# 0Setsuna0/SoftbodyUnity

Measured on AMD Instinct MI355X. Metric: particle-substeps/sec, higher is better.
Workload: dtype f32

## Files before the change

softbodyunity_amd/csrc/abi.hip:

```cpp
#include "solver_internal.hpp"

using namespace sbi;

extern "C" {

void sb_desc_default(sb_desc *d) {
    if (!d) return;
    std::memset(d, 0, sizeof(*d));
    d->world = 1;
    d->gravity[1] = -9.81f;
    d->tile_particles = 0;
    d->use_graph = 1;
}

int sb_create(const sb_desc *desc, sb_solver **out) {
    if (!desc || !out) return fail(SB_ERR_INVALID_ARG, "sb_create: null argument");
    *out = nullptr;
    return guarded([&]() -> int {
        sb_desc d = *desc;
        if (d.world <= 0) d.world = 1;
        if (d.rank < 0 || d.rank >= d.world) return fail(SB_ERR_INVALID_ARG, "sb_create: rank out of range");
        if (!(d.damping >= 0.0f)) return fail(SB_ERR_INVALID_ARG, "sb_create: damping must be >= 0");
        if (d.tile_particles > sbp::kMaxTileLocal) return fail(SB_ERR_INVALID_ARG, "sb_create: tile_particles too large");
        if (d.partition < SB_PARTITION_AUTO || d.partition > SB_PARTITION_RCB) return fail(SB_ERR_INVALID_ARG, "sb_create: partition must be SB_PARTITION_AUTO, _BLOCKS or _RCB");
// ... 464 lines not shown
    return guarded([&]() -> int {
        int rc = set_device(s); if (rc) return rc;
        HIP_CHECK(hipEventRecord(s->ev1, s->stream));
        HIP_CHECK(hipEventSynchronize(s->ev1));
        HIP_CHECK(hipEventElapsedTime(ms, s->ev0, s->ev1));
        return SB_OK;
    });
}

int sb_get_stats(sb_solver *s, sb_stats *out) {
    if (!s || !out) return fail(SB_ERR_INVALID_ARG, "sb_get_stats: null argument");
    if (!s->finalized) return fail(SB_ERR_STATE, "sb_get_stats before sb_finalize");
    std::memset(out, 0, sizeof(*out));
    const sbp::Plan &P = s->plan->plan;
    const sbp::LocalPlan &L = s->plan->local;
    out->n_particles_owned = s->n_owned;
    out->n_particles_local = s->n_local;
    for (size_t k = 0; k < L.order_mask[0].size(); ++k) if (L.order_mask[0][k]) ++out->n_constraints_local[P.order_type[0][k]];
    out->n_tilings = P.tiling ? 2 : 1;
    out->n_global_colours = (int32_t)P.gcolours.size();
    for (int tl = 0; tl < 2; ++tl) { out->n_tiles[tl] = s->tiling[tl].n_tiles; out->tile_constraints[tl] = s->tiling[tl].n_slots; }
    out->n_t2_layers = (int64_t)s->t2_layer_range.size();
    out->n_t2_tiles = s->tiling[2].n_tiles;
    out->t2_constraints = s->tiling[2].n_slots;
    out->constraints_in_tiles = P.cons_in_tiles;
    out->constraints_in_global = P.cons_in_global;
    for (size_t slot = 0; slot < s->halos.size(); ++slot) {
        const int64_t cnt = s->halos[slot]->send_off.back();
        if (slot == 1) out->halo_particles_t1 = cnt; else out->halo_particles_global += cnt;
    }
    out->device_bytes = s->dev_bytes;
    {
        const int64_t mb = s->w_uniform ? 0 : (s->w_palette ? 1 : 4);
        auto tables = [&](const DevTiling &D) { return D.stream_bytes + (int64_t)D.n_tiles * (int64_t)sizeof(sbk::TileDesc) + (int64_t)D.runs_overflow.count * 8; };
        for (int tl = 0; tl < 2; ++tl) {
            const DevTiling &D = s->tiling[tl];
            if (!D.n_tiles) continue;
            out->launch_bytes[tl] = D.staged_particles * (12 + mb + 12 + 12 + 12) + tables(D);
        }
        const DevTiling &D0 = s->tiling[0];
        if (D0.n_tiles) {
            out->launch_bytes[2] = D0.staged_particles * (12 + mb + 12 + 12 + 12) + tables(D0);
            out->launch_bytes[3] = D0.staged_particles * (12 + mb + 12 + 12 + 12) + tables(D0);
        }
        const DevTiling &D2 = s->tiling[2];
        if (D2.n_tiles) out->launch_bytes[4] = D2.staged_particles * (4 + 12 + mb + 12) + tables(D2);
    }
    out->partition = P.partition;
    out->halo_schedule = s->schedule;
    out->halo_unpack_fused = s->fused_unpack ? 1 : 0;
    out->halo_auto_state = s->calib.state;
    out->halo_auto_ticks = s->calib.n[0] + s->calib.n[1];
    out->halo_auto_ms[0] = s->calib.decided_ms[0]; out->halo_auto_ms[1] = s->calib.decided_ms[1];
    out->readback_peeks = s->n_peeks;
    out->readback_peek_tiles = s->n_peek_tiles;
    out->ticks_fused = s->n_fused;
    out->ticks_fused_kinematic = s->n_kin_fused;
    for (int tl = 0; tl < 2; ++tl) out->lane_packed_tiles[tl] = s->tiling[tl].n_packed_tiles;
    out->plan_hash = s->plan_hash;
    if (!P.rank_cost.empty()) {
        out->partition_cost = P.rank_cost[(size_t)s->desc.rank];
        for (int64_t c : P.rank_cost) { out->partition_cost_total += c; out->partition_cost_max = std::max(out->partition_cost_max, c); }
    }
    {
        std::vector<uint8_t> is_peer((size_t)s->desc.world, 0);
        for (const auto &H : s->halos) {
            for (int pr : H->peers) is_peer[(size_t)pr] = 1;
            out->halo_particles_recv += H->recv_off.back();
        }
        for (uint8_t b : is_peer) out->halo_peers += b;
    }
    return SB_OK;
}

}
```

softbodyunity_amd/csrc/device_math.hip.hpp:

```cpp
#pragma once
#include "kernel_types.hpp"

namespace sbk {

__device__ __forceinline__ float4 pv_load(const PosView &P, int g) {
    const size_t o = 3 * (size_t)g;
    return make_float4(P.xyz[o], P.xyz[o + 1], P.xyz[o + 2], P.w[g]);
}
__device__ __forceinline__ void pv_store(const PosView &P, int g, const float4 &v) {
    const size_t o = 3 * (size_t)g;
    P.xyz[o] = v.x; P.xyz[o + 1] = v.y; P.xyz[o + 2] = v.z;
}

__device__ __forceinline__ void store3_through(float *p, float x, float y, float z) {
    f32x3_t v = {x, y, z};
    asm volatile("global_store_dwordx3 %0, %1, off sc0 sc1" ::"v"(p), "v"(v) : "memory");
}

struct V3 { float x, y, z; };
__device__ __forceinline__ V3 sub3(V3 a, V3 b) { return {a.x - b.x, a.y - b.y, a.z - b.z}; }
__device__ __forceinline__ V3 cross3(V3 a, V3 b) {
    float t0 = a.y * b.z, t1 = a.z * b.y, t2 = a.z * b.x, t3 = a.x * b.z, t4 = a.x * b.y, t5 = a.y * b.x;
    return {t0 - t1, t2 - t3, t4 - t5};
}
__device__ __forceinline__ float dot3(V3 a, V3 b) {
    float xx = a.x * b.x, yy = a.y * b.y, zz = a.z * b.z;
    return (xx + yy) + zz;
}
__device__ __forceinline__ V3 addscaled3(V3 x, float s, V3 g) {
    float a = s * g.x, b = s * g.y, c = s * g.z;
    return {x.x + a, x.y + b, x.z + c};
}
__device__ __forceinline__ V3 xyz(float4 p) { return {p.x, p.y, p.z}; }

__device__ __forceinline__ float sqrt_rn_normal(float x) {
#ifdef SB_LIBM_SQRT
    return sqrtf(x);
#endif
    float s = __builtin_amdgcn_sqrtf(x);
    float sd = __int_as_float(__float_as_int(s) - 1), su = __int_as_float(__float_as_int(s) + 1);
    float rd = __builtin_fmaf(-sd, s, x), ru = __builtin_fmaf(-su, s, x);
    s = rd <= 0.0f ? sd : s;
    return ru > 0.0f ? su : s;
}

__device__ __forceinline__ bool project_distance(float4 &a, float4 &b, float L0, float at) {
    float dx = a.x - b.x, dy = a.y - b.y, dz = a.z - b.z;
    float xx = dx * dx, yy = dy * dy, zz = dz * dz;
    float L2 = (xx + yy) + zz;
// ... 220 lines not shown
```

softbodyunity_amd/csrc/kernel_types.hpp:

```cpp
#pragma once
#include <hip/hip_runtime.h>
#include <stdint.h>

#include "stream_codec.hpp"

namespace sbk {

struct TickParams {
    float h, inv_h, hgx, hgy, hgz, kd, at_d, at_v, at_b;
    float pnx, pny, pnz, pd;
    int32_t plane_on;
    float pad[2];
};

constexpr int kKindFirst = 0, kKindMid = 1, kKindLast = 2, kKindLayer = 3, kKindPeek = 4, kKindMidKinematic = 5;
constexpr bool kind_is_kinematic(int k) { return k == kKindMidKinematic; }
constexpr int kind_base(int k) { return kind_is_kinematic(k) ? kKindMid : k; }
constexpr bool kind_has_mark(int k) { return k != kKindLayer; }
constexpr bool kind_rounds_before_mark(int k) { return k != kKindFirst; }
constexpr bool kind_rounds_after_mark(int k) { return k == kKindFirst || kind_base(k) == kKindMid; }
constexpr bool kind_ends_tick(int k) { return k == kKindLast || k == kKindPeek; }
constexpr bool kind_reads_prev(int k) { return kind_base(k) == kKindMid || k == kKindLast; }
constexpr bool kind_writes_peek(int k) { return k == kKindPeek; }
constexpr bool kind_may_read_ghosts(int k) { return k == kKindMid || k == kKindLast; }
constexpr bool kind_gathers(int k) { return k == kKindLayer; }

struct TileDesc {
    int32_t n_local, run_count, n_rounds;
    int32_t gather_begin;
    uint32_t s_begin;
    uint32_t s_hdr;
    uint32_t s_len;
    uint32_t packed_lanes;
    int32_t run_overflow;
    int32_t n_pal;
    int32_t n_steps;
    uint32_t s_items;
    int2 runs[10];
};
constexpr int kInlineRuns = 10;
constexpr int kWide8MaxTiles = 768;
#ifndef SB_REG_ROUNDS
#define SB_REG_ROUNDS 4
#endif
#ifndef SB_REG_ROUNDS_NARROW
#define SB_REG_ROUNDS_NARROW 3
#endif
constexpr int kRegRoundsWide = SB_REG_ROUNDS, kRegRoundsNarrow = SB_REG_ROUNDS_NARROW;
#ifdef SB_REG_COMPACT_ONLY
constexpr bool kRegFullSlots = false;
#else
constexpr bool kRegFullSlots = true;
#endif
constexpr bool kLanePackDecodable = kRegRoundsNarrow >= kLanePackRounds;
constexpr int kMaxRoundsLds = 128;

typedef float f32x3_t __attribute__((ext_vector_type(3)));
struct PosView {
    float *xyz;
    const float *w;
};

constexpr int kMaxMassPalette = 64;

struct TileArgs {
    PosView pos;
    const uint8_t *w8;
    const float *wpal;
    float *prev;
    float *vel;
    const TileDesc *tiles;
    const int2 *runs_overflow;
    const uint32_t *stream;
    const TickParams *tp;
    const int32_t *gather;
    int32_t max_local;
    int32_t rounds_dwords;
    int32_t pal_dwords;
    int32_t win_dwords;
    int32_t tile_base;
    int32_t w_uniform;
    int32_t item_waves;
    int32_t store_through;
    const float *ghost_src;
    int32_t n_owned;
    float *peek_out;
    const int32_t *kin_map;
    float *kin_target;
};
constexpr int kHaloNone = 0, kHaloGhosts = 1;

constexpr int kNarrowTileThreads = 128;
constexpr int kQuadTileThreads = 512;
constexpr int kWideTileThreads = 256;
constexpr int kRoundSlots = 256;
constexpr int kSmallTile = 512, kLargeTile = 1024;
typedef float f32x3 __attribute__((ext_vector_type(3)));

typedef float f32x4 __attribute__((ext_vector_type(4)));
typedef uint32_t u32x4 __attribute__((ext_vector_type(4)));

constexpr int kMaxPeers = 8;
struct PeerSlot {
    int32_t n_send, n_recv;
    int32_t send_off[kMaxPeers + 1];
    int32_t send_cap[kMaxPeers];
    float *remote_data[kMaxPeers];
    int32_t remote_stride[kMaxPeers];
    int32_t my_stride[kMaxPeers];
    int32_t recv_off[kMaxPeers + 1];
    int32_t recv_cnt[kMaxPeers];
    const float *my_data[kMaxPeers];
    uint32_t *remote_data_flag[kMaxPeers];
    uint32_t *my_ack_flag[kMaxPeers];
    uint32_t *my_data_flag[kMaxPeers];
    uint32_t *remote_ack_flag[kMaxPeers];
    uint32_t *local;
// ... 13 lines not shown
```

softbodyunity_amd/csrc/launch_shape.hpp:

```cpp
#pragma once
#include "kernel_types.hpp"
#include "tables_host.hpp"

namespace sbt {

struct LaunchShape { int threads, ppt; bool quads; };
inline bool same_width(const LaunchShape &a, const LaunchShape &b) { return a.threads == b.threads && a.ppt == b.ppt; }

constexpr LaunchShape kShapeNarrow{sbk::kNarrowTileThreads, sbk::kSmallTile / sbk::kNarrowTileThreads, false};
constexpr LaunchShape kShapeWide{sbk::kWideTileThreads, sbk::kSmallTile / sbk::kWideTileThreads, false};
constexpr LaunchShape kShapeWideLarge{sbk::kWideTileThreads, sbk::kLargeTile / sbk::kWideTileThreads, false};
constexpr LaunchShape kShapeEight{sbk::kQuadTileThreads, sbk::kSmallTile / sbk::kQuadTileThreads, false};
constexpr LaunchShape kShapeEightLarge{sbk::kQuadTileThreads, sbk::kLargeTile / sbk::kQuadTileThreads, false};

inline LaunchShape tile_launch_shape(const TilingScalars &D, int tile_lanes, int quad_lanes, int narrow_min_tiles, int n_tiles_in_launch, bool ghosts) {
    const bool small = D.max_local <= sbk::kSmallTile;
    const bool narrow = small && (D.packed_lanes ? D.packed_lanes == sbk::kLanePackLanes : (tile_lanes ? tile_lanes == sbk::kNarrowTileThreads : n_tiles_in_launch >= narrow_min_tiles));
    const bool quad8 = D.has_quads && quad_lanes == sbk::kQuadTileThreads;
    const bool wide8 = small && !D.has_quads && !D.packed_lanes && (tile_lanes ? tile_lanes == sbk::kQuadTileThreads : n_tiles_in_launch <= sbk::kWide8MaxTiles);
    const bool quads = ghosts ? false : D.has_quads;
    LaunchShape sh = quads && quad8 ? (small ? kShapeEight : kShapeEightLarge) : wide8 ? kShapeEight : narrow ? kShapeNarrow : small ? kShapeWide : kShapeWideLarge;
    sh.quads = quads;
    return sh;
}

}
```

softbodyunity_amd/csrc/schedule.hip:

```cpp
#include "solver_internal.hpp"
#include "launch_shape.hpp"
#include "tile_kernel.hip.hpp"
#include "aux_kernels.hip.hpp"

namespace sbi {

sbk::TickParams tick_params(const sb_solver *s, float dt, int substeps) {
    sbk::TickParams t{};
    volatile float S = (float)substeps;
    volatile float h = dt / S;
    t.h = h;
    volatile float inv_h = 1.0f / h;
    t.inv_h = inv_h;
    volatile float hx = h * s->desc.gravity[0], hy = h * s->desc.gravity[1], hz = h * s->desc.gravity[2];
    t.hgx = hx; t.hgy = hy; t.hgz = hz;
    volatile float td = s->desc.damping * h;
    volatile float kd = 1.0f - td;
    t.kd = kd < 0.0f ? 0.0f : (float)kd;
    volatile float h2 = h * h;
    volatile float ad = s->mesh->kind[0].compliance / h2;
    volatile float av = s->mesh->kind[1].compliance / h2;
    volatile float av36 = 36.0f * av;
    volatile float ab = s->mesh->kind[2].compliance / h2;
    t.at_d = ad; t.at_v = av36; t.at_b = ab;
// ... 128 lines not shown
    if (free_list.empty()) e.create(); else { e = std::move(free_list.back()); free_list.pop_back(); }
    HIP_CHECK(hipEventRecord(e, st));
    (join ? join_pending : pending).push_back(std::move(e));
}
void ExchangeTimer::recycle() {
    for (auto *v : {&pending, &join_pending}) {
        free_list.insert(free_list.end(), std::make_move_iterator(v->begin()), std::make_move_iterator(v->end()));
        v->clear();
    }
}

void halo_exchange(sb_solver *s, int slot, hipStream_t st) {
    if (!st) st = s->stream;
    if (!halo_slot_active(s, slot)) return;
    const bool timed = s->xtimer.enabled && !s->capturing;
    if (timed) s->xtimer.mark(st);
    if (!s->peer.enabled) halo_exchange_pre(s, slot, st);
    if (timed) s->xtimer.mark(st);
    if (s->peer.enabled) halo_exchange_pre(s, slot, st);
    if (!s->peer.enabled) {
        NCCL_CHECK(rccl().GroupStart());
        try {
            halo_exchange_calls(s, slot, st);
        } catch (...) {
            (void)rccl().GroupEnd();
            throw;
        }
        NCCL_CHECK(rccl().GroupEnd());
    }
    halo_exchange_post(s, slot, st);
    if (timed) s->xtimer.mark(st);
}

template <int KIND, bool Q, int THREADS, int PPT, bool W, int G>
void launch_tile_kernel(const sb_solver *s, const DevTiling &D, const sbk::TileDesc *tiles_at_base, int n_wg, const sbk::TileArgs &A) {
    hipLaunchKernelGGL((sbk::tile_kernel<KIND, Q, THREADS, PPT, W, G>), dim3(n_wg), dim3(THREADS), D.lds_bytes + s->lds_pad, s->stream, tiles_at_base, n_wg, A);
}
template <int KIND, bool Q, bool W, int G>
void launch_tile_shaped(const sb_solver *s, const DevTiling &D, const sbt::LaunchShape &sh, const sbk::TileDesc *tiles_at_base, int n_wg, const sbk::TileArgs &A) {
    using namespace sbt;
    if (same_width(sh, kShapeEight)) return launch_tile_kernel<KIND, Q, kShapeEight.threads, kShapeEight.ppt, W, G>(s, D, tiles_at_base, n_wg, A);
    if constexpr (Q) if (same_width(sh, kShapeEightLarge)) return launch_tile_kernel<KIND, Q, kShapeEightLarge.threads, kShapeEightLarge.ppt, W, G>(s, D, tiles_at_base, n_wg, A);
    if (same_width(sh, kShapeNarrow)) return launch_tile_kernel<KIND, Q, kShapeNarrow.threads, kShapeNarrow.ppt, W, G>(s, D, tiles_at_base, n_wg, A);
    if (same_width(sh, kShapeWide)) return launch_tile_kernel<KIND, Q, kShapeWide.threads, kShapeWide.ppt, W, G>(s, D, tiles_at_base, n_wg, A);
    if (same_width(sh, kShapeWideLarge)) return launch_tile_kernel<KIND, Q, kShapeWideLarge.threads, kShapeWideLarge.ppt, W, G>(s, D, tiles_at_base, n_wg, A);
    throw std::runtime_error("internal: no tile kernel is built for the launch shape asked for");
}

template <int KIND>
void launch_tile(sb_solver *s, DevTiling &D, int tile_begin = 0, int tile_end = -1, int halo = sbk::kHaloNone, const sbk::TileDesc *table = nullptr) {
    const bool ghosts = halo == sbk::kHaloGhosts;
    if (tile_end < 0) tile_end = D.n_tiles;
    if (tile_end <= tile_begin) return;
    sbk::TileArgs A{};
    A.pos = s->pos_view(); A.w8 = s->d_w8.p; A.wpal = s->d_wpal.p; A.prev = s->d_prev.p; A.vel = s->d_vel.p;
    A.tiles = D.tiles.p; A.runs_overflow = D.runs_overflow.p; A.stream = D.stream.p;
    A.tp = s->d_tp.p;
    A.gather = D.gather.p;
    A.w_uniform = s->w_uniform ? 1 : 0;
    A.item_waves = D.item_waves;
    A.store_through = tile_end - tile_begin <= s->store_through_max_tiles ? 3 : s->store_through_large;
    A.ghost_src = ghosts ? s->d_recvbuf.p : nullptr; A.n_owned = (int32_t)s->n_owned;
    A.peek_out = sbk::kind_writes_peek(KIND) ? s->d_peek.p : nullptr;
    A.kin_map = sbk::kind_is_kinematic(KIND) ? s->d_kin_map.p : nullptr; A.kin_target = sbk::kind_is_kinematic(KIND) ? s->d_kin_target.p : nullptr;
    A.max_local = D.max_local; A.win_dwords = D.win_dwords; A.tile_base = tile_begin; A.pal_dwords = D.pal_dwords; A.rounds_dwords = D.rounds_dwords;
    const sbk::TileDesc *tiles_at_base = table ? table : D.tiles.p + tile_begin;
    const int n_wg = tile_end - tile_begin;
    const sbt::LaunchShape sh = sbt::tile_launch_shape(D, s->tile_lanes, s->quad_lanes, s->narrow_min_tiles, n_wg, ghosts);
    constexpr bool kCanGhost = sbk::kind_may_read_ghosts(KIND);
    if (ghosts && !(kCanGhost && !D.has_quads)) throw std::runtime_error("internal: ghost-reading tile kernel requested for a launch that has none");
    const bool W = s->w_palette;
    if (ghosts) {
        if constexpr (kCanGhost) W ? launch_tile_shaped<KIND, false, true, sbk::kHaloGhosts>(s, D, sh, tiles_at_base, n_wg, A) : launch_tile_shaped<KIND, false, false, sbk::kHaloGhosts>(s, D, sh, tiles_at_base, n_wg, A);
    } else if (sh.quads) W ? launch_tile_shaped<KIND, true, true, sbk::kHaloNone>(s, D, sh, tiles_at_base, n_wg, A) : launch_tile_shaped<KIND, true, false, sbk::kHaloNone>(s, D, sh, tiles_at_base, n_wg, A);
    else W ? launch_tile_shaped<KIND, false, true, sbk::kHaloNone>(s, D, sh, tiles_at_base, n_wg, A) : launch_tile_shaped<KIND, false, false, sbk::kHaloNone>(s, D, sh, tiles_at_base, n_wg, A);
}

struct LaunchTimer {
    std::vector<Event> ev;
    std::vector<int> slot;
    hipStream_t stream;
    void begin(int which) {
        Event a, b;
        a.create(); b.create();
        HIP_CHECK(hipEventRecord(a, stream));
        ev.push_back(std::move(a)); ev.push_back(std::move(b)); slot.push_back(which);
    }
    void end() { HIP_CHECK(hipEventRecord(ev.back(), stream)); }
};

void launch_tick_kernel(sb_solver *s, int it, int substeps, LaunchTimer *lt, int tile_begin = 0, int tile_end = -1, bool kin = false) {
    const int tl = s->plan->plan.tiling ? (it & 1) : 0;
    DevTiling &D = s->tiling[tl];
    if (lt && D.n_tiles) lt->begin(it == 0 ? 2 + (int)s->gcolours.size() : (it == substeps ? 3 + (int)s->gcolours.size() : tl));
    const int halo_in = s->fused_unpack && tl == 1 ? sbk::kHaloGhosts : sbk::kHaloNone;
    if (it == 0) launch_tile<sbk::kKindFirst>(s, D, tile_begin, tile_end);
    else if (it < substeps && kin) launch_tile<sbk::kKindMidKinematic>(s, D, tile_begin, tile_end);
    else if (it < substeps) launch_tile<sbk::kKindMid>(s, D, tile_begin, tile_end, halo_in);
    else launch_tile<sbk::kKindLast>(s, D, tile_begin, tile_end, halo_in);
    if (lt && D.n_tiles) lt->end();
}

void launch_t2_layer(sb_solver *s, int layer, LaunchTimer *lt, bool with_halo = true) {
    const auto rg = s->t2_layer_range[layer];
// ... 434 lines not shown
```

softbodyunity_amd/csrc/solver_internal.hpp:

```cpp
#pragma once
#include <hip/hip_runtime.h>
#include <rccl/rccl.h>
#include <dlfcn.h>

#include <algorithm>
#include <array>
#include <atomic>
#include <chrono>
#include <climits>
#include <cmath>
#include <cstdio>
#include <cstdlib>
#include <cstring>
#include <limits>
#include <map>
#include <memory>
#include <mutex>
#include <type_traits>
#include <stdexcept>
#include <string>
#include <utility>
#include <vector>

#include "../../include/softbody.h"
// ... 108 lines not shown
struct sb_plan {
    sbp::Plan plan;
    sbp::LocalPlan local;
    bool owns_local = true;
};

struct sb_solver {
    sb_desc desc;
    bool finalized = false;
    sbi::Stream stream;
    sbi::Event ev0, ev1;
    ncclComm_t comm = nullptr;
    bool loopback = false;
    int schedule = SB_SCHEDULE_SERIAL_EAGER;
    uint64_t plan_hash = 0;
    sbi::Stream comm_stream;
    sbi::Event ev_boundary, ev_halo;
    bool overlap_halo = false;
    std::shared_ptr<sbi::AuthoredMesh> mesh = std::make_shared<sbi::AuthoredMesh>();
    bool sharded = false;
    sb_domain domain{};
    std::vector<int32_t> global_id;
    std::unique_ptr<sb_plan> plan;
    int64_t dev_bytes = 0;
    int64_t n_owned = 0, n_local = 0;
    DevBuf<float> d_pos3;
    DevBuf<float> d_wf;
    DevBuf<uint8_t> d_w8;
    DevBuf<float> d_wpal;
    bool w_palette = false;
    bool w_uniform = false;
    sbk::PosView pos_view() const { return sbk::PosView{d_pos3.p, d_wf.p}; }
    DevBuf<float> d_prev, d_vel;
    DevBuf<sbk::TickParams> d_tp;
    DevBuf<float> d_sendbuf, d_recvbuf;
    DevTiling tiling[3];
    std::vector<std::pair<int32_t, int32_t>> t2_layer_range;
    std::vector<std::unique_ptr<DevGColour>> gcolours;
    std::vector<std::unique_ptr<DevHalo>> halos;
    sbk::TickParams tp_host{};
    bool tp_valid = false;
    sbi::GraphCache graphs;
    bool deferred = false;
    int deferred_substeps = 0;
    uint32_t tune_flags = 0;
    int win_dwords_cap = 0;
    int prev_offset_bytes = 0;
    bool lazy_tick = true;
    int tile_lanes = 0;
    int quad_lanes = 512;
    int store_through_max_tiles = 6144;
    int store_through_large = 0;
    int narrow_min_tiles = 10240;
    size_t lds_pad = 0;
    bool pack_tiles = true;
    bool fused_unpack = false;
    bool graph_rccl = false;
    std::vector<float> h_stage;
    struct AutoSchedule {
        int state = 0;
        int tick = 0;
        sbi::Event ev[8];
        int n[2] = {0, 0};
        double decided_ms[2] = {0, 0};
    } calib;
    bool group_walk = false;
// ... 129 lines not shown
```

softbodyunity_amd/csrc/tables.hip:

```cpp
#include "solver_internal.hpp"

namespace sbi {

sbp::Input make_input(const float *rest, int32_t n, const int32_t *d, int64_t md, const int32_t *v, int64_t mv,
                      const int32_t *b, int64_t mb) {
    sbp::Input in;
    in.rest = rest; in.n = n; in.dist_ij = d; in.m_d = md; in.vol = v; in.m_v = mv; in.bend = b; in.m_b = mb;
    return in;
}

sbp::Domain to_domain(const sb_domain &d) {
    sbp::Domain D;
    D.set = true; D.n_global = d.n_global; D.ell = d.spacing; D.fill = d.fill > 0 && d.fill <= 1 ? d.fill : 1.0;
    for (int a = 0; a < 3; ++a) { D.lo[a] = d.lo[a]; D.hi[a] = d.hi[a]; }
    return D;
}
sbp::Opts plan_opts(int rank, int world, const int32_t dims[3], int32_t tile_particles, int32_t partition, uint32_t plan_flags,
                    int64_t m_v, int64_t m_b, const sb_domain *domain) {
    sbp::Opts o;
    if (domain) {
        o.domain = to_domain(*domain);
        if (domain->four_vertex_constraints) m_v += 1;
    }
    o.rank = rank; o.world = world <= 0 ? 1 : world;
    for (int a = 0; a < 3; ++a) o.dims[a] = dims ? dims[a] : 0;
    o.tile_particles = tile_particles != 0 ? tile_particles : (m_v + m_b > 0 ? 256 : 512);
    o.partition = partition;
    o.third_tiling = !(plan_flags & SB_PLAN_NO_T2);
    o.third_list = !(plan_flags & SB_PLAN_NO_THIRD_LIST);
    o.cluster_layers = !(plan_flags & SB_PLAN_NO_CLUSTER_LAYERS);
    o.mixed_groups = !(plan_flags & SB_PLAN_NO_MIXED_GROUPS);
    o.bank_aware_lanes = !(plan_flags & SB_PLAN_NO_BANK_ORDER);
    o.merge_tiles = !(plan_flags & SB_PLAN_NO_TILE_MERGE);
// ... 75 lines not shown
    HIP_CHECK(hipMemset(s->d_prev.p, 0, (size_t)s->n_local * 3 * sizeof(float)));
    s->d_tp.alloc(1, s->dev_bytes);
    for (int tl = 0; tl < 3; ++tl) {
        sbt::build_tiling(in, opt, tl, H);
        sbt::HostTiling &T = H.T[tl];
        DevTiling &D = s->tiling[tl];
        static_cast<sbt::TilingScalars &>(D) = T;
        D.tiles.upload(T.tiles, s->dev_bytes); D.runs_overflow.upload(T.runs_overflow, s->dev_bytes);
        D.stream.upload(T.stream, s->dev_bytes);
        D.gather.upload(T.gather, s->dev_bytes);
        T.release_arrays();
    }
    s->t2_layer_range = H.t2_layer_range;
    sbt::build_gcolours(in, H);
    for (const sbt::HostGColour &G : H.gcolours) {
        auto D = std::make_unique<DevGColour>();
        D->type = G.type; D->count = G.count;
        if (G.type == 0) { D->ij.upload(G.ij, s->dev_bytes); D->rest.upload(G.rest, s->dev_bytes); }
        else { D->quad.upload(G.quad, s->dev_bytes); D->rest2.upload(G.rest2, s->dev_bytes); }
        s->gcolours.push_back(std::move(D));
    }
    sbt::build_halos(in, opt, H);
    for (sbt::HostHalo &G : H.halos) {
        auto D = std::make_unique<DevHalo>();
        D->send_idx.upload(G.send_idx, s->dev_bytes); D->recv_idx.upload(G.recv_idx, s->dev_bytes);
        D->peers = std::move(G.peers); D->send_off = std::move(G.send_off); D->recv_off = std::move(G.recv_off);
        s->halos.push_back(std::move(D));
    }
    s->d_sendbuf.alloc(H.send_floats, s->dev_bytes);
    s->d_recvbuf.alloc(H.recv_floats, s->dev_bytes);
    if (H.recv_floats) HIP_CHECK(hipMemset(s->d_recvbuf.p, 0, H.recv_floats * sizeof(float)));
    s->fused_unpack = H.fused_unpack;
    if (s->peer.enabled && L.world > 1) alloc_mailbox(s, H.mailbox);
}

}
```

softbodyunity_amd/csrc/tile_kernel.hip.hpp:

```cpp
#pragma once
#include "device_math.hip.hpp"

namespace sbk {

__device__ __forceinline__ void lds_barrier() { asm volatile("s_waitcnt lgkmcnt(0)\n\ts_barrier" ::: "memory"); }

__device__ __forceinline__ void decode_compact_distance(uint32_t e, const float *s_pal, int &i, int &k, float &L0) { i = compact_slot_i(e); k = compact_slot_j(e); L0 = s_pal[compact_slot_pal(e)]; }
__device__ __forceinline__ void decode_full_distance(const uint2 e, int &i, int &k, float &L0) { i = pair_i(e.x); k = pair_j(e.x); L0 = __uint_as_float(e.y); }
__device__ __forceinline__ void read_distance_slot(const uint32_t *slots, int c, bool compact, const float *s_pal, int &i, int &k, float &L0) {
    if (compact) decode_compact_distance(slots[c], s_pal, i, k, L0);
    else decode_full_distance(*reinterpret_cast<const uint2 *>(slots + kFullSlotDwords * c), i, k, L0);
}

__device__ __forceinline__ void quad_slot_offsets(const uint4 &e, int q, int &o0, int &o1, int &o2, int &o3) {
    o0 = 4 * (int)pair_i(e.x) + q; o1 = 4 * (int)pair_j(e.x) + q;
    o2 = 4 * (int)pair_i(e.y) + q; o3 = 4 * (int)pair_j(e.y) + q;
}

template <bool QUADS, int THREADS> constexpr int kWavesPerSimd = QUADS ? (THREADS == 64 ? 3 : (THREADS == 512 ? 2 : 4)) : (THREADS == 256 ? 8 : (THREADS == 128 ? 6 : 4));
template <int KIND_, bool QUADS, int THREADS, int PPT, bool WPAL, int HALO = kHaloNone>
__global__ __launch_bounds__(THREADS, (kWavesPerSimd<QUADS, THREADS> - (KIND_ == 5 && !QUADS ? 1 : 0))) void tile_kernel(const TileDesc *tiles_at_base, int n_workgroups, TileArgs A) {
    constexpr int KIND = kind_base(KIND_);
    constexpr bool KIN = kind_is_kinematic(KIND_);
    constexpr bool GHOSTS = HALO == kHaloGhosts;
    constexpr int kTileThreads = THREADS;
    constexpr int kCPL = THREADS >= kRoundSlots ? 1 : kRoundSlots / THREADS;
    extern __shared__ uint4 lds_raw[];
    float4 *lds_pos = reinterpret_cast<float4 *>(lds_raw);
    uint32_t *s_rounds = reinterpret_cast<uint32_t *>(lds_pos + A.max_local);
    float *s_pal = reinterpret_cast<float *>(s_rounds + A.rounds_dwords);
    uint32_t *cbuf = s_rounds + A.rounds_dwords + A.pal_dwords;
    f32x3 *lds_spare = reinterpret_cast<f32x3 *>(cbuf + A.win_dwords);
    typedef const TileDesc __attribute__((address_space(4))) *ConstTileDescPtr;
#ifndef SB_NO_XCD_REMAP
    const int nwg = n_workgroups, wg = (int)blockIdx.x;
    const int xq = nwg >> 3, xr = nwg & 7, xcd = wg & 7;
    const int tile_index = (xcd < xr ? xcd * (xq + 1) : xr * (xq + 1) + (xcd - xr) * xq) + (wg >> 3);
#else
    const int tile_index = (int)blockIdx.x;
#endif
    const TileDesc __attribute__((address_space(4))) &td = *((ConstTileDescPtr)(uintptr_t)tiles_at_base + tile_index);
    const int n_rounds_all = td.n_rounds;
    const int tid = threadIdx.x;
    const int n_local = td.n_local;
    const int run_count = td.run_count;
    const TickParams tp = *A.tp;
    const uint32_t *tstream = A.stream + td.s_begin;
#if defined(SB_ABLATE) && SB_ABLATE == 4
    if (n_local >= 0) { if (n_rounds_all == 0x7fffffff) A.vel[0] = tp.h; return; }
#endif

    int g[PPT];
    if (kind_gathers(KIND_)) {
// ... 19 lines not shown
                    if (rn.y <= l) gi = rn.x + (l - rn.y);
                }
            g[m] = l < n_local ? gi : -1;
        }
    }
    const int R = n_rounds_all;
    const int v_begin = kind_rounds_before_mark(KIND_) ? 0 : R;
    const int v_end = !kind_has_mark(KIND_) ? R : (kind_rounds_after_mark(KIND_) ? 2 * R + 1 : R + 1);
    const uint32_t d_lo = td.s_hdr;
    const uint32_t d_hi = td.s_len;
    const uint32_t win = (uint32_t)A.win_dwords;
    uint32_t win_lo = d_lo;
    auto load_window = [&](uint32_t lo) {
        const uint32_t n4 = (min(lo + win, d_hi) - lo) >> 2;
        const uint4 *src = reinterpret_cast<const uint4 *>(tstream + lo);
        uint4 *dst = reinterpret_cast<uint4 *>(cbuf);
        uint32_t t0 = (uint32_t)tid;
        asm volatile("" : "+v"(t0));
        for (uint32_t i = t0; i < n4; i += 4 * kTileThreads) {
            uint4 v0 = src[i], v1, v2, v3;
            const bool b1 = i + kTileThreads < n4, b2 = i + 2 * kTileThreads < n4, b3 = i + 3 * kTileThreads < n4;
            if (b1) v1 = src[i + kTileThreads];
            if (b2) v2 = src[i + 2 * kTileThreads];
            if (b3) v3 = src[i + 3 * kTileThreads];
            dst[i] = v0;
            if (b1) dst[i + kTileThreads] = v1;
            if (b2) dst[i + 2 * kTileThreads] = v2;
            if (b3) dst[i + 3 * kTileThreads] = v3;
        }
    };
    f32x4 X[PPT];
    float pvx[PPT], pvy[PPT], pvz[PPT];
    uint32_t wi[PPT];
    const int mypal = WPAL ? __float_as_int(A.wpal[tid & (kMaxMassPalette - 1)]) : 0;
#pragma unroll
    for (int m = 0; m < PPT; ++m) {
        const int gc = max(g[m], 0);
        const bool ghost = GHOSTS && gc >= A.n_owned;
        const float *px = ghost ? A.ghost_src + 6 * (size_t)(gc - A.n_owned) : A.pos.xyz + 3 * (size_t)gc;
        X[m].x = px[0]; X[m].y = px[1]; X[m].z = px[2];
        if (WPAL) { wi[m] = A.w8[A.w_uniform ? 0 : gc]; X[m].w = 0.0f; } else { wi[m] = 0; X[m].w = A.pos.w[gc]; }
        pvx[m] = pvy[m] = pvz[m] = 0.0f;
        if (kind_reads_prev(KIND_)) {
            const float *pp = ghost ? px + 3 : A.prev + 3 * (size_t)gc;
            pvx[m] = pp[0]; pvy[m] = pp[1]; pvz[m] = pp[2];
        }
    }
    const bool rounds_in_lds = n_rounds_all <= A.rounds_dwords;
    const uint32_t rw = tstream[max(min(tid, n_rounds_all - 1), 0)];
    const bool rounds_in_lanes = n_rounds_all <= 64;
    const uint32_t rwl = tstream[max(min(tid & 63, n_rounds_all - 1), 0)];
    uint32_t itreg = 0;
    if (QUADS && kTileThreads == 64 * A.item_waves) {
        const int ns = td.n_steps;
        itreg = tstream[ns > 0 ? td.s_items + (uint32_t)((tid >> 6) * ns + min(tid & 63, ns - 1)) : 0u];
    }
    const int n_pal = td.n_pal;
    const uint32_t palw = tstream[tid < n_pal ? ((n_rounds_all + 3) & ~3) + tid : 0];
#ifndef SB_KW
#define SB_KW (QUADS ? 4 : 2)
#endif
    constexpr int kW = SB_KW;
    const bool lane_packed = !QUADS && kTileThreads == kLanePackLanes && td.packed_lanes == (uint32_t)kLanePackLanes;
    const bool lane_packed_full = !WPAL && lane_packed && td.n_pal == 0;
    const bool wide_packed = !QUADS && kTileThreads == kWidePackLanes && td.packed_lanes == (uint32_t)kWidePackLanes;
    const bool any_packed = lane_packed || wide_packed;
    const uint32_t n4_first = wide_packed ? 0u : lane_packed ? (lane_packed_full ? 2u * (uint32_t)kLanePackLanes : (uint32_t)kLanePackLanes)
                                          : (min(win_lo + win, d_hi) - win_lo) >> 2;
    const u32x4 *wsrc = reinterpret_cast<const u32x4 *>(tstream + win_lo);
    u32x4 wv[kW];
#pragma unroll
    for (int q = 0; q < kW; ++q) {
        const uint32_t i = tid + q * kTileThreads;
        wv[q] = i < n4_first ? wsrc[i] : *reinterpret_cast<const u32x4 *>(tstream);
    }
    typedef uint32_t u32x2 __attribute__((ext_vector_type(2)));
    u32x2 wc = {0u, 0u};
    u32x2 wp = {0u, 0u};
    if (!QUADS && kTileThreads == kWidePackLanes)
        wp = *reinterpret_cast<const u32x2 *>(wide_packed ? tstream + win_lo + 2u * (uint32_t)tid : tstream);
#pragma unroll
    for (int m = 0; m < PPT; ++m) asm volatile("" ::"v"(X[m].x), "v"(pvx[m]), "v"(wi[m]), "v"(X[m].w));
    asm volatile("" ::"v"(mypal));
    if (WPAL) {
#pragma unroll
        for (int m = 0; m < PPT; ++m) X[m].w = __int_as_float(__builtin_amdgcn_ds_bpermute((int)(wi[m] << 2), mypal));
    }
#pragma unroll
    for (int q = 0; q < kW; ++q) asm volatile("" ::"v"(wv[q].x));
    asm volatile("" ::"v"(rw), "v"(palw), "v"(rwl), "v"(itreg));
    if (!QUADS && kTileThreads == kWidePackLanes) asm volatile("" ::"v"(wp.x));
#pragma unroll
    for (int m = 0; m < PPT; ++m)
        if (g[m] >= 0) *reinterpret_cast<f32x4 *>(lds_pos + tid + m * kTileThreads) = X[m];
    if (rounds_in_lds && tid < n_rounds_all) s_rounds[tid] = rw;
    if (tid < n_pal) s_pal[tid] = __uint_as_float(palw);
    if (kTileThreads < kMaxRoundsLds && rounds_in_lds)
        for (int q = tid + kTileThreads; q < n_rounds_all; q += kTileThreads) s_rounds[q] = tstream[q];
    if (kTileThreads < kMaxPalette)
        for (int q = tid + kTileThreads; q < n_pal; q += kTileThreads) s_pal[q] = __uint_as_float(tstream[((n_rounds_all + 3) & ~3) + q]);
    {
        u32x4 *dst = reinterpret_cast<u32x4 *>(cbuf);
#pragma unroll
        for (int q = 0; q < kW; ++q) {
            const uint32_t i = tid + q * kTileThreads;
            if (i < n4_first && !any_packed) dst[i] = wv[q];
        }
        if (!any_packed)
            for (uint32_t i = tid + kW * kTileThreads; i < n4_first; i += kTileThreads) dst[i] = wsrc[i];
    }
    __syncthreads();
    if (!WPAL && !QUADS && kTileThreads == kLanePackLanes && lane_packed_full)
        wc = *reinterpret_cast<const u32x2 *>(tstream + win_lo + 8u * (uint32_t)kLanePackLanes + 2u * (uint32_t)tid);
#if defined(SB_ABLATE) && SB_ABLATE == 5
    if (n_local >= 0) { if (lds_pos[tid].x == 1.2345e-30f && cbuf[tid] == 0x12345678u) A.vel[0] = tp.h; return; }
#endif
// ... 5 lines not shown
                const int l = tid + m * kTileThreads;
                float4 P = lds_pos[l];
                if (KIND != kKindFirst && tp.plane_on && P.w > 0.0f) {
                    float a = tp.pnx * P.x, b = tp.pny * P.y, c = tp.pnz * P.z;
                    float pen = ((a + b) + c) - tp.pd;
                    if (pen < 0.0f) {
                        float dx = pen * tp.pnx, dy = pen * tp.pny, dz = pen * tp.pnz;
                        P.x = P.x - dx; P.y = P.y - dy; P.z = P.z - dz;
                        if (kind_ends_tick(KIND_)) lds_pos[l] = P;
                    }
                }
                if (KIND == kKindPeek) continue;
                float vx, vy, vz;
                const size_t o = 3 * (size_t)g[m];
                if (KIND == kKindFirst) {
                    vx = A.vel[o + 0]; vy = A.vel[o + 1]; vz = A.vel[o + 2];
                } else {
                    float dx = P.x - pvx[m], dy = P.y - pvy[m], dz = P.z - pvz[m];
                    float qx = dx * tp.inv_h, qy = dy * tp.inv_h, qz = dz * tp.inv_h;
                    vx = qx * tp.kd; vy = qy * tp.kd; vz = qz * tp.kd;
                }
                bool moved = false;
                if (KIN && P.w == 0.0f) {
                    const int ks = A.kin_map[g[m]];
                    if (ks >= 0) {
                        float *t = A.kin_target + 3 * (size_t)ks;
                        const float tx = t[0], ty = t[1], tz = t[2];
                        if (tx == tx) { P.x = tx; P.y = ty; P.z = tz; moved = true; t[0] = __int_as_float(0x7fc00000); }
                    }
                }
                if (KIND == kKindLast) {
                    A.vel[o + 0] = vx; A.vel[o + 1] = vy; A.vel[o + 2] = vz;
                } else {
                    if (A.store_through & 1) store3_through(A.prev + o, P.x, P.y, P.z);
                    else { A.prev[o + 0] = P.x; A.prev[o + 1] = P.y; A.prev[o + 2] = P.z; }
                    if (P.w > 0.0f) {
                        vx = vx + tp.hgx; vy = vy + tp.hgy; vz = vz + tp.hgz;
                        float hx = tp.h * vx, hy = tp.h * vy, hz = tp.h * vz;
                        P.x = P.x + hx; P.y = P.y + hy; P.z = P.z + hz;
                        lds_pos[l] = P;
                    } else if (KIN && moved) lds_pos[l] = P;
                }
            }
    };

    constexpr int kRegRounds = THREADS >= 256 ? kRegRoundsWide : kRegRoundsNarrow;
    if (kRegRounds > 0 && !QUADS && n_rounds_all <= kRegRounds && n_rounds_all > 0 && (kRegFullSlots || n_pal > 0) && (any_packed || d_hi - d_lo <= win)) {
        const bool tile_compact = n_pal > 0;
        uint32_t rs[kRegRounds > 0 ? kRegRounds : 1][kCPL];
        float rl[kRegRounds > 0 ? kRegRounds : 1][kCPL];
        int rcnt[kRegRounds > 0 ? kRegRounds : 1];
        {
            uint32_t o = 0;
#pragma unroll
            for (int r = 0; r < kRegRounds; ++r) {
                rcnt[r] = 0;
                if (r < n_rounds_all) {
                    rcnt[r] = (int)group_dist_count((uint32_t)__builtin_amdgcn_readlane((int)rwl, r));
                    if (kCPL == 2 && lane_packed) {
#pragma unroll
                        for (int u = 0; u < kCPL; ++u) {
                            const int bit = kLanePackFieldBits * (2 * r + u), w0 = bit >> 5, sh = bit & 31;
                            const uint32_t lo = wv[0][w0] >> sh;
                            const uint32_t hi = (sh + kLanePackFieldBits > 32) ? (wv[0][w0 + 1 < kLaneWordDwords ? w0 + 1 : kLaneWordDwords - 1] << ((32 - sh) & 31)) : 0u;
                            const uint32_t f = (lo | hi) & kLanePackFieldMask;
                            rs[r][u] = compact_slot_of_pack_field(f);
                            if (!WPAL) {
// ... 249 lines not shown
            for (int u = 0; u < kCPL; ++u) {
                ca[u] = *reinterpret_cast<const f32x4 *>(lds_pos + ci[u]);
                cb[u] = *reinterpret_cast<const f32x4 *>(lds_pos + ck[u]);
            }
#pragma unroll
            for (int u = 0; u < kCPL; ++u) {
                float4 a = make_float4(ca[u].x, ca[u].y, ca[u].z, ca[u].w), b = make_float4(cb[u].x, cb[u].y, cb[u].z, cb[u].w);
                con[u] = project_distance_nobranch(a, b, cL0[u], tp.at_d) && con[u];
                ca[u].x = a.x; ca[u].y = a.y; ca[u].z = a.z; cb[u].x = b.x; cb[u].y = b.y; cb[u].z = b.z;
            }
#pragma unroll
            for (int u = 0; u < kCPL; ++u) {
                f32x3 *da = con[u] ? reinterpret_cast<f32x3 *>(lds_pos + ci[u]) : lds_spare;
                f32x3 *db = con[u] ? reinterpret_cast<f32x3 *>(lds_pos + ck[u]) : lds_spare;
                *da = (f32x3){ca[u].x, ca[u].y, ca[u].z};
                *db = (f32x3){cb[u].x, cb[u].y, cb[u].z};
            }
        }
        off += size;
#if defined(SB_ABLATE) && SB_ABLATE == 3
        asm volatile("s_waitcnt lgkmcnt(0)" ::: "memory");
#else
        lds_barrier();
#endif
    }
    }
#pragma unroll
    for (int m = 0; m < PPT; ++m)
        if (g[m] >= 0) {
            const float4 P = lds_pos[tid + m * kTileThreads];
            if (kind_writes_peek(KIND_)) { float *o = A.peek_out + 3 * (size_t)g[m]; o[0] = P.x; o[1] = P.y; o[2] = P.z; }
            else if (A.store_through & 2) store3_through(A.pos.xyz + 3 * (size_t)g[m], P.x, P.y, P.z);
            else pv_store(A.pos, g[m], P);
        }
}


}
```

Before: 115.4 billion.

## Encode previous positions as 64-bit bit-deltas against current positions

Replaces the 12-byte previous-position array with an 8-byte code per particle. The code packs 21-bit signed deltas between the float bit patterns of the previous and current positions, with an escape flag that falls back to the full-precision prev array when a delta does not fit. It is enabled only for single-rank, palette-mass, narrow spring-only tilings with no intermediate steps, and aims to cut memory traffic in the bandwidth-bound tile kernels. The cost is extra encode/decode ALU work, a divergent fallback path, and a restricted set of configurations where it applies.

```diff
diff --git a/softbodyunity_amd/csrc/abi.hip b/softbodyunity_amd/csrc/abi.hip
--- a/softbodyunity_amd/csrc/abi.hip
+++ b/softbodyunity_amd/csrc/abi.hip
@@ -520,16 +520,17 @@
     out->device_bytes = s->dev_bytes;
     {
         const int64_t mb = s->w_uniform ? 0 : (s->w_palette ? 1 : 4);
+        const int64_t pb = s->prev_codes ? 8 : 12;
         auto tables = [&](const DevTiling &D) { return D.stream_bytes + (int64_t)D.n_tiles * (int64_t)sizeof(sbk::TileDesc) + (int64_t)D.runs_overflow.count * 8; };
         for (int tl = 0; tl < 2; ++tl) {
             const DevTiling &D = s->tiling[tl];
             if (!D.n_tiles) continue;
-            out->launch_bytes[tl] = D.staged_particles * (12 + mb + 12 + 12 + 12) + tables(D);
+            out->launch_bytes[tl] = D.staged_particles * (12 + mb + pb + 12 + pb) + tables(D);
         }
         const DevTiling &D0 = s->tiling[0];
         if (D0.n_tiles) {
-            out->launch_bytes[2] = D0.staged_particles * (12 + mb + 12 + 12 + 12) + tables(D0);
-            out->launch_bytes[3] = D0.staged_particles * (12 + mb + 12 + 12 + 12) + tables(D0);
+            out->launch_bytes[2] = D0.staged_particles * (12 + mb + 12 + 12 + pb) + tables(D0);
+            out->launch_bytes[3] = D0.staged_particles * (12 + mb + pb + 12 + 12) + tables(D0);
         }
         const DevTiling &D2 = s->tiling[2];
         if (D2.n_tiles) out->launch_bytes[4] = D2.staged_particles * (4 + 12 + mb + 12) + tables(D2);
diff --git a/softbodyunity_amd/csrc/device_math.hip.hpp b/softbodyunity_amd/csrc/device_math.hip.hpp
--- a/softbodyunity_amd/csrc/device_math.hip.hpp
+++ b/softbodyunity_amd/csrc/device_math.hip.hpp
@@ -15,6 +15,10 @@
 __device__ __forceinline__ void store3_through(float *p, float x, float y, float z) {
     f32x3_t v = {x, y, z};
     asm volatile("global_store_dwordx3 %0, %1, off sc0 sc1" ::"v"(p), "v"(v) : "memory");
+}
+typedef uint32_t u32x2_t __attribute__((ext_vector_type(2)));
+__device__ __forceinline__ void store2_through(uint2 *p, u32x2_t v) {
+    asm volatile("global_store_dwordx2 %0, %1, off sc0 sc1" ::"v"(p), "v"(v) : "memory");
 }
 
 struct V3 { float x, y, z; };
diff --git a/softbodyunity_amd/csrc/kernel_types.hpp b/softbodyunity_amd/csrc/kernel_types.hpp
--- a/softbodyunity_amd/csrc/kernel_types.hpp
+++ b/softbodyunity_amd/csrc/kernel_types.hpp
@@ -21,6 +21,7 @@
 constexpr bool kind_rounds_after_mark(int k) { return k == kKindFirst || kind_base(k) == kKindMid; }
 constexpr bool kind_ends_tick(int k) { return k == kKindLast || k == kKindPeek; }
 constexpr bool kind_reads_prev(int k) { return kind_base(k) == kKindMid || k == kKindLast; }
+constexpr bool kind_touches_prev(int k) { return k == kKindFirst || kind_reads_prev(k); }
 constexpr bool kind_writes_peek(int k) { return k == kKindPeek; }
 constexpr bool kind_may_read_ghosts(int k) { return k == kKindMid || k == kKindLast; }
 constexpr bool kind_gathers(int k) { return k == kKindLayer; }
@@ -82,7 +83,10 @@
     int32_t w_uniform;
     int32_t item_waves;
     int32_t store_through;
-    const float *ghost_src;
+    union {
+        const float *ghost_src;
+        uint2 *prev_code;
+    };
     int32_t n_owned;
     float *peek_out;
     const int32_t *kin_map;
diff --git a/softbodyunity_amd/csrc/launch_shape.hpp b/softbodyunity_amd/csrc/launch_shape.hpp
--- a/softbodyunity_amd/csrc/launch_shape.hpp
+++ b/softbodyunity_amd/csrc/launch_shape.hpp
@@ -24,4 +24,25 @@
     return sh;
 }
 
+inline bool tiling_always_narrow(const TilingScalars &D, int tile_lanes) {
+    if (D.n_tiles == 0) return true;
+    return D.max_local <= sbk::kSmallTile && !D.has_quads && (D.packed_lanes ? D.packed_lanes == sbk::kLanePackLanes : tile_lanes == sbk::kNarrowTileThreads);
 }
+constexpr int64_t kPrevCodeMaxParticles = (int64_t)1 << 26;
+struct PrevCodeInputs {
+    int world = 1;
+    int halo_slots = 0;
+    int tile_lanes = 0;
+    bool w_palette = false;
+    int steps_between_tiles = 0;
+    int64_t n_local = 0;
+};
+inline bool use_prev_codes(const TilingScalars &T0, const TilingScalars &T1, const PrevCodeInputs &in) {
+    if (in.world != 1 || in.halo_slots != 0) return false;
+    if (!in.w_palette) return false;
+    if (in.steps_between_tiles != 0) return false;
+    if (T0.n_tiles == 0 || in.n_local > kPrevCodeMaxParticles) return false;
+    return tiling_always_narrow(T0, in.tile_lanes) && tiling_always_narrow(T1, in.tile_lanes);
+}
+
+}
diff --git a/softbodyunity_amd/csrc/prev_code.hpp b/softbodyunity_amd/csrc/prev_code.hpp
--- /dev/null
+++ b/softbodyunity_amd/csrc/prev_code.hpp
@@ -0,0 +1,34 @@
+#pragma once
+#include <stdint.h>
+
+#ifdef __HIPCC__
+#define SB_PREV_FN __host__ __device__ __forceinline__
+#else
+#define SB_PREV_FN inline
+#endif
+
+namespace sbk {
+
+constexpr int kPrevFieldBits = 21;
+constexpr uint32_t kPrevFieldMask = (1u << kPrevFieldBits) - 1u, kPrevHalf = 1u << (kPrevFieldBits - 1);
+constexpr uint64_t kPrevEscape = 1ull << 63;
+
+struct Bits3 { uint32_t x, y, z; };
+struct PrevCode { uint64_t code; bool fits; };
+
+SB_PREV_FN bool prev_delta_fits(uint32_t k) { return k + kPrevHalf < 2u * kPrevHalf; }
+SB_PREV_FN bool prev_is_escape(uint64_t code) { return (code >> 63) != 0; }
+SB_PREV_FN bool prev_hi_is_escape(uint32_t code_hi) { return (code_hi >> 31) != 0; }
+SB_PREV_FN PrevCode prev_encode(Bits3 P, Bits3 x) {
+    const uint32_t kx = P.x - x.x, ky = P.y - x.y, kz = P.z - x.z;
+    const bool fits = prev_delta_fits(kx) && prev_delta_fits(ky) && prev_delta_fits(kz);
+    const uint64_t f = (uint64_t)(kx & kPrevFieldMask) | ((uint64_t)(ky & kPrevFieldMask) << kPrevFieldBits) | ((uint64_t)(kz & kPrevFieldMask) << (2 * kPrevFieldBits));
+    return {fits ? f : kPrevEscape, fits};
+}
+SB_PREV_FN uint32_t prev_field_delta(uint32_t f) { return (f ^ kPrevHalf) - kPrevHalf; }
+SB_PREV_FN Bits3 prev_decode(uint64_t code, Bits3 x) {
+    const uint32_t fx = (uint32_t)code & kPrevFieldMask, fy = (uint32_t)(code >> kPrevFieldBits) & kPrevFieldMask, fz = (uint32_t)(code >> (2 * kPrevFieldBits)) & kPrevFieldMask;
+    return {x.x + prev_field_delta(fx), x.y + prev_field_delta(fy), x.z + prev_field_delta(fz)};
+}
+
+}
diff --git a/softbodyunity_amd/csrc/schedule.hip b/softbodyunity_amd/csrc/schedule.hip
--- a/softbodyunity_amd/csrc/schedule.hip
+++ b/softbodyunity_amd/csrc/schedule.hip
@@ -184,9 +184,9 @@
     if (timed) s->xtimer.mark(st);
 }
 
-template <int KIND, bool Q, int THREADS, int PPT, bool W, int G>
+template <int KIND, bool Q, int THREADS, int PPT, bool W, int G, bool C = false>
 void launch_tile_kernel(const sb_solver *s, const DevTiling &D, const sbk::TileDesc *tiles_at_base, int n_wg, const sbk::TileArgs &A) {
-    hipLaunchKernelGGL((sbk::tile_kernel<KIND, Q, THREADS, PPT, W, G>), dim3(n_wg), dim3(THREADS), D.lds_bytes + s->lds_pad, s->stream, tiles_at_base, n_wg, A);
+    hipLaunchKernelGGL((sbk::tile_kernel<KIND, Q, THREADS, PPT, W, G, C>), dim3(n_wg), dim3(THREADS), D.lds_bytes + s->lds_pad, s->stream, tiles_at_base, n_wg, A);
 }
 template <int KIND, bool Q, bool W, int G>
 void launch_tile_shaped(const sb_solver *s, const DevTiling &D, const sbt::LaunchShape &sh, const sbk::TileDesc *tiles_at_base, int n_wg, const sbk::TileArgs &A) {
@@ -222,6 +222,11 @@
     constexpr bool kCanGhost = sbk::kind_may_read_ghosts(KIND);
     if (ghosts && !(kCanGhost && !D.has_quads)) throw std::runtime_error("internal: ghost-reading tile kernel requested for a launch that has none");
     const bool W = s->w_palette;
+    if constexpr (sbk::kind_touches_prev(KIND)) if (s->prev_codes) {
+        if (ghosts || sh.quads || !W || !sbt::same_width(sh, sbt::kShapeNarrow)) throw std::runtime_error("internal: previous-position codes are on, but the launch is not 128 x 4 spring-only with palette masses");
+        A.prev_code = s->d_prev_code.p;
+        return launch_tile_kernel<KIND, false, sbt::kShapeNarrow.threads, sbt::kShapeNarrow.ppt, true, sbk::kHaloNone, true>(s, D, tiles_at_base, n_wg, A);
+    }
     if (ghosts) {
         if constexpr (kCanGhost) W ? launch_tile_shaped<KIND, false, true, sbk::kHaloGhosts>(s, D, sh, tiles_at_base, n_wg, A) : launch_tile_shaped<KIND, false, false, sbk::kHaloGhosts>(s, D, sh, tiles_at_base, n_wg, A);
     } else if (sh.quads) W ? launch_tile_shaped<KIND, true, true, sbk::kHaloNone>(s, D, sh, tiles_at_base, n_wg, A) : launch_tile_shaped<KIND, true, false, sbk::kHaloNone>(s, D, sh, tiles_at_base, n_wg, A);
diff --git a/softbodyunity_amd/csrc/solver_internal.hpp b/softbodyunity_amd/csrc/solver_internal.hpp
--- a/softbodyunity_amd/csrc/solver_internal.hpp
+++ b/softbodyunity_amd/csrc/solver_internal.hpp
@@ -164,6 +164,8 @@
     bool w_uniform = false;
     sbk::PosView pos_view() const { return sbk::PosView{d_pos3.p, d_wf.p}; }
     DevBuf<float> d_prev, d_vel;
+    bool prev_codes = false;
+    DevBuf<uint2> d_prev_code;
     DevBuf<sbk::TickParams> d_tp;
     DevBuf<float> d_sendbuf, d_recvbuf;
     DevTiling tiling[3];
diff --git a/softbodyunity_amd/csrc/tables.hip b/softbodyunity_amd/csrc/tables.hip
--- a/softbodyunity_amd/csrc/tables.hip
+++ b/softbodyunity_amd/csrc/tables.hip
@@ -1,4 +1,5 @@
 #include "solver_internal.hpp"
+#include "launch_shape.hpp"
 
 namespace sbi {
 
@@ -140,6 +141,16 @@
     if (H.recv_floats) HIP_CHECK(hipMemset(s->d_recvbuf.p, 0, H.recv_floats * sizeof(float)));
     s->fused_unpack = H.fused_unpack;
     if (s->peer.enabled && L.world > 1) alloc_mailbox(s, H.mailbox);
+    sbt::PrevCodeInputs pc;
+    pc.world = s->desc.world; pc.tile_lanes = s->tile_lanes; pc.w_palette = s->w_palette; pc.n_local = s->n_local;
+    pc.halo_slots = s->loopback ? 1 : 0;
+    for (const auto &D : s->halos) if (D->active()) ++pc.halo_slots;
+    pc.steps_between_tiles = (int)s->t2_layer_range.size() + (int)s->gcolours.size();
+    s->prev_codes = sbt::use_prev_codes(s->tiling[0], s->tiling[1], pc);
+    if (s->prev_codes) {
+        s->d_prev_code.alloc((size_t)s->n_local, s->dev_bytes);
+        HIP_CHECK(hipMemset(s->d_prev_code.p, 0, (size_t)s->n_local * sizeof(uint2)));
+    }
 }
 
 }
diff --git a/softbodyunity_amd/csrc/tile_kernel.hip.hpp b/softbodyunity_amd/csrc/tile_kernel.hip.hpp
--- a/softbodyunity_amd/csrc/tile_kernel.hip.hpp
+++ b/softbodyunity_amd/csrc/tile_kernel.hip.hpp
@@ -1,5 +1,6 @@
 #pragma once
 #include "device_math.hip.hpp"
+#include "prev_code.hpp"
 
 namespace sbk {
 
@@ -18,7 +19,7 @@
 }
 
 template <bool QUADS, int THREADS> constexpr int kWavesPerSimd = QUADS ? (THREADS == 64 ? 3 : (THREADS == 512 ? 2 : 4)) : (THREADS == 256 ? 8 : (THREADS == 128 ? 6 : 4));
-template <int KIND_, bool QUADS, int THREADS, int PPT, bool WPAL, int HALO = kHaloNone>
+template <int KIND_, bool QUADS, int THREADS, int PPT, bool WPAL, int HALO = kHaloNone, bool CODED = false>
 __global__ __launch_bounds__(THREADS, (kWavesPerSimd<QUADS, THREADS> - (KIND_ == 5 && !QUADS ? 1 : 0))) void tile_kernel(const TileDesc *tiles_at_base, int n_workgroups, TileArgs A) {
     constexpr int KIND = kind_base(KIND_);
     constexpr bool KIN = kind_is_kinematic(KIND_);
@@ -104,6 +105,7 @@
     f32x4 X[PPT];
     float pvx[PPT], pvy[PPT], pvz[PPT];
     uint32_t wi[PPT];
+    uint32_t pc_lo[PPT], pc_hi[PPT];
     const int mypal = WPAL ? __float_as_int(A.wpal[tid & (kMaxMassPalette - 1)]) : 0;
 #pragma unroll
     for (int m = 0; m < PPT; ++m) {
@@ -113,9 +115,13 @@
         X[m].x = px[0]; X[m].y = px[1]; X[m].z = px[2];
         if (WPAL) { wi[m] = A.w8[A.w_uniform ? 0 : gc]; X[m].w = 0.0f; } else { wi[m] = 0; X[m].w = A.pos.w[gc]; }
         pvx[m] = pvy[m] = pvz[m] = 0.0f;
+        pc_lo[m] = pc_hi[m] = 0u;
         if (kind_reads_prev(KIND_)) {
-            const float *pp = ghost ? px + 3 : A.prev + 3 * (size_t)gc;
-            pvx[m] = pp[0]; pvy[m] = pp[1]; pvz[m] = pp[2];
+            if (CODED) { const uint2 c = A.prev_code[gc]; pc_lo[m] = c.x; pc_hi[m] = c.y; }
+            else {
+                const float *pp = ghost ? px + 3 : A.prev + 3 * (size_t)gc;
+                pvx[m] = pp[0]; pvy[m] = pp[1]; pvz[m] = pp[2];
+            }
         }
     }
     const bool rounds_in_lds = n_rounds_all <= A.rounds_dwords;
@@ -152,8 +158,28 @@
     if (!QUADS && kTileThreads == kWidePackLanes)
         wp = *reinterpret_cast<const u32x2 *>(wide_packed ? tstream + win_lo + 2u * (uint32_t)tid : tstream);
 #pragma unroll
-    for (int m = 0; m < PPT; ++m) asm volatile("" ::"v"(X[m].x), "v"(pvx[m]), "v"(wi[m]), "v"(X[m].w));
+    for (int m = 0; m < PPT; ++m) {
+        if (CODED) asm volatile("" ::"v"(X[m].x), "v"(pc_lo[m]), "v"(wi[m]), "v"(X[m].w));
+        else asm volatile("" ::"v"(X[m].x), "v"(pvx[m]), "v"(wi[m]), "v"(X[m].w));
+    }
     asm volatile("" ::"v"(mypal));
+    if (CODED && kind_reads_prev(KIND_)) {
+        bool esc = false;
+#pragma unroll
+        for (int m = 0; m < PPT; ++m) {
+            const Bits3 p = prev_decode((uint64_t)pc_lo[m] | ((uint64_t)pc_hi[m] << 32), Bits3{__float_as_uint(X[m].x), __float_as_uint(X[m].y), __float_as_uint(X[m].z)});
+            pvx[m] = __uint_as_float(p.x); pvy[m] = __uint_as_float(p.y); pvz[m] = __uint_as_float(p.z);
+            esc = esc || (g[m] >= 0 && prev_hi_is_escape(pc_hi[m]));
+        }
+        if (__builtin_amdgcn_ballot_w64(esc) != 0ull) {
+#pragma unroll
+            for (int m = 0; m < PPT; ++m)
+                if (g[m] >= 0 && prev_hi_is_escape(pc_hi[m])) {
+                    const float *pp = A.prev + 3 * (size_t)g[m];
+                    pvx[m] = pp[0]; pvy[m] = pp[1]; pvz[m] = pp[2];
+                }
+        }
+    }
     if (WPAL) {
 #pragma unroll
         for (int m = 0; m < PPT; ++m) X[m].w = __int_as_float(__builtin_amdgcn_ds_bpermute((int)(wi[m] << 2), mypal));
@@ -225,7 +251,8 @@
                 if (KIND == kKindLast) {
                     A.vel[o + 0] = vx; A.vel[o + 1] = vy; A.vel[o + 2] = vz;
                 } else {
-                    if (A.store_through & 1) store3_through(A.prev + o, P.x, P.y, P.z);
+                    if (CODED) { pvx[m] = P.x; pvy[m] = P.y; pvz[m] = P.z; }
+                    else if (A.store_through & 1) store3_through(A.prev + o, P.x, P.y, P.z);
                     else { A.prev[o + 0] = P.x; A.prev[o + 1] = P.y; A.prev[o + 2] = P.z; }
                     if (P.w > 0.0f) {
                         vx = vx + tp.hgx; vy = vy + tp.hgy; vz = vz + tp.hgz;
@@ -541,6 +568,17 @@
             if (kind_writes_peek(KIND_)) { float *o = A.peek_out + 3 * (size_t)g[m]; o[0] = P.x; o[1] = P.y; o[2] = P.z; }
             else if (A.store_through & 2) store3_through(A.pos.xyz + 3 * (size_t)g[m], P.x, P.y, P.z);
             else pv_store(A.pos, g[m], P);
+            if (CODED && kind_has_mark(KIND_) && !kind_ends_tick(KIND_)) {
+                const PrevCode e = prev_encode(Bits3{__float_as_uint(pvx[m]), __float_as_uint(pvy[m]), __float_as_uint(pvz[m])}, Bits3{__float_as_uint(P.x), __float_as_uint(P.y), __float_as_uint(P.z)});
+                const u32x2_t c = {(uint32_t)e.code, (uint32_t)(e.code >> 32)};
+                if (A.store_through & 1) store2_through(A.prev_code + g[m], c);
+                else *reinterpret_cast<u32x2_t *>(A.prev_code + g[m]) = c;
+                if (!e.fits) {
+                    float *o = A.prev + 3 * (size_t)g[m];
+                    if (A.store_through & 1) store3_through(o, pvx[m], pvy[m], pvz[m]);
+                    else { o[0] = pvx[m]; o[1] = pvy[m]; o[2] = pvz[m]; }
+                }
+            }
         }
 }
 
```

After: 123.9 billion, median of 6. 7.3% higher.
